# JJanai/slowflow

Measured on AMD Instinct MI355X. Metric: Mpix*solver-iters/s at 1024x436 (whole coarse-to-fine path), higher is better.
Workload: dtype f32

## Files before the change

### slowflow_amd/csrc/api.hip

```cpp
#include <algorithm>
#include <cmath>
#include <cstring>
#include <memory>
#include <mutex>

#include "sfa_internal.h"

#pragma clang fp contract(off)

namespace sfa {

thread_local std::string g_thread_err;

#ifndef SFA_RELEASE
Switches g_switches;
#endif
#ifndef SFA_RELEASE
static const char *const kSwitchNames[Switches::N] = {
    "SFA_SOR_CHAIN", "SFA_SOR_BAND", "SFA_SOR_F", "SFA_SOR_CH", "SFA_SOR_LEAD", "SFA_CHAIN_LDS", "SFA_RB_TILE", "SFA_WARP_ALLJ", "SFA_NO_WARP_SMOOTH",
    "SFA_ASSEMBLE_GENERIC", "SFA_EXACT_DIV", "SFA_ASM_XCD", "SFA_NO_DIRECT_OPERANDS", "SFA_NO_UV_ALIAS", "SFA_DEBUG_ACTIVE", "SFA_UNFUSED", "SFA_SHARE_SOR",
    "SFA_PYRAMID_UNFUSED", "SFA_CUT_DISCHARGE", "SFA_CUT_INNER", "SFA_CUT_SUPER", "SFA_CUT_TAIL_INNER", "SFA_CUT_PER", "SFA_CUT_TAIL_PER", "SFA_CUT_TAIL_SUPER",
    "SFA_CUT_DEBUG", "SFA_CUT_NO_TAIL", "SFA_CUT_TAIL", "SFA_NO_EXACT_BREAK"};
static int set_switch(const char *name, const char *value) {
    for (int i = 0; i < Switches::N; i++)
        if (!strcmp(name, kSwitchNames[i])) {
            g_switches.given[i] = value != nullptr;
            g_switches.value[i] = value ? atoi(value) : 0;
            return SFA_OK;
        }
    return SFA_ERR_ARG;
}
static void switches_from_environment() {
    static std::once_flag once;
    std::call_once(once, [] {
        const char *d = getenv("SFA_DEBUG");
        if (!d || atoi(d) == 0) return;
        for (int i = 0; i < Switches::N; i++)
            if (const char *e = getenv(kSwitchNames[i])) (void)set_switch(kSwitchNames[i], e);
    });
}
#else
static void switches_from_environment() {}
#endif

int set_error(sfa_ctx *ctx, int code, const char *fmt, ...) {
// ... 58 lines not shown
    float *warp(int s, int sp1) const { return base + off_warp + (long)(s + sp1) * 3 * pl; }
    float *frame(int f) const { return pbase + 2 * pl + (long)f * 3 * pl; }
    float *tmp() const { return base + off_tmp; }
    Geo geo() const { return Geo{w, h, pitch, pl, es, nb, WMask::first(nb), nullptr}; }
    Geo geo(const WMask &active) const { return Geo{w, h, pitch, pl, es, nb, active, nullptr}; }
    static long persistent_floats(int pitch, int h, int ref) { return (long)pitch * h * (2 + (2L * ref + 1) * 3); }
    static long transient_floats(int pitch, int h, int ref, bool fused) {
        return (long)pitch * h * ((P_COUNT - 2) + 2 * ref + (2L * ref + 1) * 3 + (fused ? 0 : 2L * ref * 2 * 24));
    }
    void layout(float *transient, float *persistent, int w_, int h_, int lstride_, int ref_, int nb_, long es_, bool fused_) {
        base = transient; pbase = persistent; w = w_; h = h_; pitch = dev_pitch(w_); lstride = lstride_; ref = ref_; F = 2 * ref_ + 1; nb = nb_; es = es_; fused = fused_;
        pl = (long)pitch * h;
        off_masks = (long)(P_COUNT - 2) * pl;
        off_warp = off_masks + 2L * ref * pl;
        off_stacks = off_warp + (2L * ref + 1) * 3 * pl;
        off_tmp = off_warp;
    }
};

struct ChannelWeights { const float *dev = nullptr; long pl = 0, es = 0; int pitch = 0, stride0 = 0; };

static const float *pair_image(const Level &L, int s, int sp1) { return (s + sp1 - L.ref == 0) ? L.frame(s + sp1) : L.warp(s, sp1); }

static bool get_derivatives(sfa_ctx *c, const Level &L, const sfa_params &p, const Geo &g, const bool need_toref[2 * SFA_MAX_REF], bool with_smoothness = false) {
    const int ref = L.ref;
    WarpJobs J;
    J.n = 0;
    for (int f = p.one_direction ? ref + 1 : 0; f <= 2 * ref; f++) {
        if (f == ref) continue;
        const int s = f < ref ? f : f - 1;
        J.job[J.n++] = WarpJob{L.frame(f) - L.base, L.warp(f < ref ? f : f - 1, f < ref ? 0 : 1) - L.base, L.mask(s) - L.base, f - ref};
    }
    const bool smoothed = with_smoothness && L.fused &&
                          launch_warp_smooth(c, g, J, L.base, L.plane(P_WX), L.plane(P_WY), p.smoothing, L.plane(P_SH), L.plane(P_SV), L.plane(P_DPSIS), p.alpha, pen(p.robust_reg));
    if (!smoothed) launch_warp_jobs(c, g, J, L.base, L.plane(P_WX), L.plane(P_WY));
    for (int s = p.one_direction ? ref : 0; s < 2 * ref; s++) {
        if (L.fused) continue;
        const float *w_s = pair_image(L, s, 0), *w_sp1 = pair_image(L, s, 1);
        launch_deriv_stack(c, g, L.stack(s, 0), w_s, w_sp1, L.es, L.es);
        if (need_toref[s]) {
            if (s < ref) launch_deriv_stack(c, g, L.stack(s, 1), w_s, L.frame(ref), L.es, L.es);
            else         launch_deriv_stack(c, g, L.stack(s, 1), L.frame(ref), w_sp1, L.es, L.es);
        }
    }
    return smoothed;
}

static int optimize_occlusions(sfa_ctx *c, const Level &L, const sfa_params &p, const Geo &g, DevMem &scratch) {
    const int ref = L.ref;
    const size_t n = (size_t)L.nb * L.pl;
    SFA_TRY(scratch.alloc(c, (2 + kCutWorkPlanes) * n * sizeof(float)));
    float *d0 = scratch.f(), *d1 = d0 + n, *work = d1 + n;
    OccArgs oa;
    memset(&oa, 0, sizeof oa);
// ... 43 lines not shown
    AssembleArgs aa;
    memset(&aa, 0, sizeof aa);
    bool need_toref[2 * SFA_MAX_REF] = {false};
    for (int s = 0; s < ref; s++) {
        if (!p.one_direction) {
            if (p.rho[ref - 1 - s] > 0)
                aa.t[aa.n++] = Term{L.off_stacks + ((long)s * 2 + 0) * 24 * L.pl, L.off_masks + (long)s * L.pl, p.rho[ref - 1 - s] * delta_over3,
                                    p.rho[ref - 1 - s] * gamma_over3, (float)(s - ref), 0};
            if (p.omega[ref - 1 - s] > 0) {
                aa.t[aa.n++] = Term{L.off_stacks + ((long)s * 2 + 1) * 24 * L.pl, L.off_masks + (long)s * L.pl, p.omega[ref - 1 - s] * delta_over3,
                                    p.omega[ref - 1 - s] * gamma_over3, (float)(s - ref), 1};
                need_toref[s] = true;
            }
        }
        if (p.rho[s] > 0)
            aa.t[aa.n++] = Term{L.off_stacks + ((long)(ref + s) * 2 + 0) * 24 * L.pl, L.off_masks + (long)(ref + s) * L.pl, p.rho[s] * delta_over3,
                                p.rho[s] * gamma_over3, (float)s, 0};
        if (p.omega[s] > 0) {
            aa.t[aa.n++] = Term{L.off_stacks + ((long)(ref + s) * 2 + 1) * 24 * L.pl, L.off_masks + (long)(ref + s) * L.pl, p.omega[s] * delta_over3,
                                p.omega[s] * gamma_over3, (float)(s + 1), 1};
            need_toref[ref + s] = true;
        }
    }
    for (int t = 0; t < aa.n; t++) {
        Term &T = aa.t[t];
        const int slot = (int)((T.mask_off - L.off_masks) / L.pl);
        const float *i1 = pair_image(L, slot, 0), *i2 = pair_image(L, slot, 1);
        if (T.is_ref) { if (slot < ref) i2 = L.frame(ref); else i1 = L.frame(ref); }
        T.i1_off = i1 - L.base; T.i2_off = i2 - L.base; T.backward = slot < ref;
    }
    aa.data_norm = data_norm; aa.one_direction = p.one_direction;
    for (int t = 0; t < aa.n; t++)
        if (aa.t[t].is_ref && aa.t[t].s == 0) return set_error(c, SFA_ERR_REF_FRAME, "Frame compared to reference frame is the reference frame itself!");
    aa.dt_norm = p.dataterm_norm;
    aa.color = pen(p.robust_color); aa.grad = pen(p.robust_grad);
    aa.chw = cw.dev; aa.chw_pl = cw.pl; aa.chw_es = cw.es; aa.chw_pitch = cw.pitch; aa.chw_stride0 = cw.stride0; aa.lstride = L.lstride;
    aa.accumulate = 0; aa.do_laplacian = 1;

    const bool use_thres_in = p.thres_inner > 0, use_thres_out = p.thres_outer > 0;
    double *red = c->d_red;
    const double npx = (double)L.h * L.w;
    constexpr int kLag = kMaskLag, kRing = kMaskRing;
    const bool dbg = sw_given(Switches::DEBUG_ACTIVE);
    g.amask = c->d_amask;
    float *const dfa = use_thres_out && !sw_given(Switches::NO_EXACT_BREAK) ? L.plane(P_A11) : nullptr, *const dfb = dfa ? L.plane(P_A12) : nullptr;
    float *const ifa = use_thres_in && !sw_given(Switches::NO_EXACT_BREAK) ? L.plane(P_A11) : nullptr, *const ifb = ifa ? L.plane(P_A12) : nullptr;
    SFA_HIP(c, hipMemsetAsync(c->d_last, 0, sizeof(LastBlock), c->stream));
    launch_set_mask(c, all);

    for (int alter = 0; alter < p.niter_alter; alter++) {
        active = all;
        g.active = active;
        if (use_thres_out && alter > 0) launch_set_mask(c, all);
        bool smoothed = get_derivatives(c, L, p, g, need_toref, uv_alias);
        if (alter > 0 && p.occlusion_reasoning && !p.one_direction) SFA_TRY(optimize_occlusions(c, L, p, g, cut_scratch));
        if (alter > 0 && p.occlusion_reasoning && occ_log)
            launch_copy_planes(c, g, occ_log + (long)alter * L.pl, L.plane(P_OCC), 1, (long)p.niter_alter * L.pl, L.es);
        for (int outer = 0; outer < p.niter_outer; outer++) {
            if (use_thres_out && outer >= kLag) {
                const int slot = (outer - kLag) % kRing;
                SFA_HIP(c, hipEventSynchronize(c->ev_mask[slot]));
                for (int i = 0; i < kMaskWords; i++) active.w[i] = *(volatile unsigned long long *)&c->h_amask[slot].w[i];
                if (!active.any()) break;
            }
            if (dbg) fprintf(stderr, "level %dx%d alter %d outer %d known active %d\n", L.w, L.h, alter, outer, active.count());
            g.active = active;
            if (outer > 0) smoothed = get_derivatives(c, L, p, g, need_toref, uv_alias);
            if (!L.fused) launch_mask_weight(c, g, L.mask(0), L.plane(P_OCC), data_norm, ref, p.one_direction);
            const bool red_black = p.sor_order == 1;
            const bool direct_outer = L.fused && !red_black && !sw_given(Switches::NO_DIRECT_OPERANDS);
            if (!direct_outer) launch_zero_planes(c, g, L.plane(P_DU), 2);
            WMask in_active = active, outer_done = WMask::none();
            for (int inner = 0; inner < p.niter_inner; inner++) {
                Geo gi = g;
                gi.active = in_active;
                const bool direct = direct_outer;
                const bool decide_in = use_thres_in && inner + 1 < p.niter_inner && ifa;
                const bool first_zero = direct && inner == 0;
                if (!first_zero) {
                    launch_copy_planes(c, gi, L.plane(P_ODU), L.plane(P_DU), 2, L.es, L.es);
                }
                if (!(smoothed && inner == 0))
                    launch_smoothness(c, gi, p.smoothing, L.plane(P_SH), L.plane(P_SV), UU, VV, L.plane(P_DPSIS), p.alpha,
                                      pen(p.robust_reg));
                aa.op = SorOperandOut();
                aa.zero_duv = first_zero ? 1 : 0;
                if (direct) SFA_TRY(sor_operand_target(c, sorws, gi, p.niter_solver, &aa.op));
                if (L.fused)
                    SFA_TRY(launch_assemble_images(c, gi, aa, L.base, L.plane(P_A11), L.plane(P_A12), L.plane(P_A22), L.plane(P_B1), L.plane(P_B2), L.plane(P_DU),
                                                   L.plane(P_DV), UU, VV, L.plane(P_SH), L.plane(P_SV), L.plane(P_OCC)));
// ... 1079 lines not shown
```

### slowflow_amd/csrc/kernels.hip

```cpp
#include "sfa_device.h"

#pragma clang fp contract(off)

namespace sfa {

__device__ __forceinline__ float psi_vec(const PenaltyDev &p, float xsq) {
    const float e2 = p.eps * p.eps;
    switch (p.id) {
    case 0: return 1.0f;
    case 2: return __fdiv_rn(1.0f, 2.0f * e2 + xsq);
    case 3: {
        float out = __fdiv_rn(1.0f, 2.0f * sqrt_rn(xsq + e2));
        if (sqrt_rn(xsq) > p.trunc) out = 0.0f;
        return out;
    }
    case 4: {
        float t = e2 + xsq;
        t = t * t;
        return __fdiv_rn(e2 + 2.0f * xsq, t);
    }
    default: return __fdiv_rn(1.0f, 2.0f * sqrt_rn(xsq + e2));
    }
}
__device__ __forceinline__ float psi_scalar(const PenaltyDev &p, float xsq) {
// ... 6 lines not shown
        if (sqrt_rn(xsq) > p.trunc) return 0.0f;
        return __fdiv_rn(1.0f, 2.0f * sqrt_rn(xsq + e2f));
    case 4: {
        float t = (float)(e2d + (double)xsq);
        t = t * t;
        return (float)((e2d + (double)(2.0f * xsq)) / (double)t);
    }
    default: return (float)(1.0 / (2.0 * __dsqrt_rn((double)xsq + e2d)));
    }
}

__global__ void k_warp(float *__restrict__ dst3, float *__restrict__ mask, const float *__restrict__ src3, const float *__restrict__ wx,
                       const float *__restrict__ wy, Geo g, int factor, long src_es) {
    const int b = blockIdx.z;
    if (!elem_active(g, b)) return;
    const int x = blockIdx.x * BX + threadIdx.x, y = blockIdx.y * BY + threadIdx.y;
    if (x >= g.w || y >= g.h) return;
    dst3 += b * g.es; wx += b * g.es; wy += b * g.es; src3 += b * src_es;
    const size_t o = (size_t)y * g.pitch + x;
    if (factor == 0) {
        for (int k = 0; k < 3; k++) dst3[k * g.pl + o] = src3[k * g.pl + o];
        return;
    }
    const float xx = x + factor * wx[o];
    const float yy = y + factor * wy[o];
    const int xi = floor_to_int_x86(xx), yi = floor_to_int_x86(yy);
    const float dx = xx - xi, dy = yy - yi;
    if (mask) mask[b * g.es + o] = (xx >= 0 && xx <= g.w - 1 && yy >= 0 && yy <= g.h - 1) ? 1.0f : 0.0f;
    const int x1 = clampi(xi, 0, g.w - 1), x2 = clampi(xi + 1, 0, g.w - 1);
    const int y1 = clampi(yi, 0, g.h - 1), y2 = clampi(yi + 1, 0, g.h - 1);
    const float ax = 1.0f - dx, ay = 1.0f - dy;
    for (int k = 0; k < 3; k++) {
        const float *s = src3 + k * g.pl;
        dst3[k * g.pl + o] = s[(size_t)y1 * g.pitch + x1] * ax * ay + s[(size_t)y1 * g.pitch + x2] * dx * ay
                           + s[(size_t)y2 * g.pitch + x1] * ax * dy + s[(size_t)y2 * g.pitch + x2] * dx * dy;
    }
}
template <bool ALLJ>
__global__ void k_warp_jobs(WarpJobs J, float *__restrict__ base, const float *__restrict__ wx, const float *__restrict__ wy, Geo g) {
    const int b = ALLJ ? blockIdx.z : blockIdx.z / J.n, j0 = ALLJ ? 0 : blockIdx.z % J.n;
    if (!elem_active(g, b)) return;
    const int x = blockIdx.x * BX + threadIdx.x, y = blockIdx.y * BY + threadIdx.y;
    if (x >= g.w || y >= g.h) return;
    const long eb = b * g.es;
    const size_t o = (size_t)y * g.pitch + x;
    const float fx0 = wx[eb + o], fy0 = wy[eb + o];
    for (int j = j0; j <= (ALLJ ? J.n - 1 : j0); j++) {
        const int factor = J.job[j].factor;
        const float *src3 = base + eb + J.job[j].src_off;
        float *dst3 = base + eb + J.job[j].dst_off;
        const float xx = x + factor * fx0;
        const float yy = y + factor * fy0;
        const int xi = floor_to_int_x86(xx), yi = floor_to_int_x86(yy);
        const float dx = xx - xi, dy = yy - yi;
        if (J.job[j].mask_off >= 0) base[eb + J.job[j].mask_off + o] = (xx >= 0 && xx <= g.w - 1 && yy >= 0 && yy <= g.h - 1) ? 1.0f : 0.0f;
        const int x1 = clampi(xi, 0, g.w - 1), x2 = clampi(xi + 1, 0, g.w - 1);
        const int y1 = clampi(yi, 0, g.h - 1), y2 = clampi(yi + 1, 0, g.h - 1);
        const float ax = 1.0f - dx, ay = 1.0f - dy;
        float out[3];
#pragma unroll
        for (int k = 0; k < 3; k++) {
            const float *s = src3 + k * g.pl;
            out[k] = s[(size_t)y1 * g.pitch + x1] * ax * ay + s[(size_t)y1 * g.pitch + x2] * dx * ay
                   + s[(size_t)y2 * g.pitch + x1] * ax * dy + s[(size_t)y2 * g.pitch + x2] * dx * dy;
        }
#pragma unroll
        for (int k = 0; k < 3; k++) dst3[k * g.pl + o] = out[k];
    }
}
void launch_warp_jobs(sfa_ctx *c, const Geo &g, const WarpJobs &J, float *base, const float *wx, const float *wy) {
    if (J.n <= 0) return;
    const bool allj = sw_int(Switches::WARP_ALLJ, 1) != 0;
    if (allj) hipLaunchKernelGGL(k_warp_jobs<true>, grid2d(g), block2d(), 0, c->stream, J, base, wx, wy, g);
    else hipLaunchKernelGGL(k_warp_jobs<false>, grid2d(g, J.n), block2d(), 0, c->stream, J, base, wx, wy, g);
}
void launch_warp(sfa_ctx *c, const Geo &g, float *dst3, float *mask, const float *src3, const float *wx, const float *wy, int factor, long src_es) {
    hipLaunchKernelGGL(k_warp, grid2d(g), block2d(), 0, c->stream, dst3, mask, src3, wx, wy, g, factor, src_es);
}
// ... 315 lines not shown
    const unsigned pitch4 = 4u * (unsigned)g.pitch;
    const float *pu = uu_ + eb, *pv = vv_ + eb, *pd = dps_ + eb;
    for (int i = tid; i < SM_R * SM_W; i += 64 * WS_ROWS) {
        const int gx = x0 + i % SM_W, gy = y0 + i / SM_W;
        if (gx >= 0 && gx < g.w && gy >= 0 && gy < g.h) {
            const unsigned o4 = (unsigned)gy * pitch4 + 4u * (unsigned)gx;
            tU[i] = ld(pu, o4); tV[i] = ld(pv, o4); tD[i] = ld(pd, o4);
        }
    }
    __syncthreads();
    const SmTile uu{tU, x0, y0}, vv{tV, x0, y0}, dps{tD, x0, y0};
    const int w = g.w, h = g.h;
    const int x = x0 + 1 + threadIdx.x;
    sh += eb; sv += eb;
    for (int k = 0; k < SM_Y / WS_ROWS; k++) {
        const int y = y0 + 1 + threadIdx.y + WS_ROWS * k;
        if (x >= g.pitch || y >= h) continue;
        const unsigned o4 = (unsigned)y * pitch4 + 4u * (unsigned)x;
        if (x >= w) { st(sh, o4, 0.0f); st(sv, o4, 0.0f); continue; }
        const float fx0 = uu(x, y), fy0 = vv(x, y);
        auto gather = [&](int j, float(&out)[3]) {
            const int factor = J.job[j].factor;
            const float *src3 = base + eb + J.job[j].src_off;
            const float xx = x + factor * fx0;
            const float yy = y + factor * fy0;
            const int xi = floor_to_int_x86(xx), yi = floor_to_int_x86(yy);
            const float dx = xx - xi, dy = yy - yi;
            if (J.job[j].mask_off >= 0) st(base + eb + J.job[j].mask_off, o4, (xx >= 0 && xx <= g.w - 1 && yy >= 0 && yy <= g.h - 1) ? 1.0f : 0.0f);
            const int x1 = clampi(xi, 0, g.w - 1), x2 = clampi(xi + 1, 0, g.w - 1);
            const int y1 = clampi(yi, 0, g.h - 1), y2 = clampi(yi + 1, 0, g.h - 1);
            const float ax = 1.0f - dx, ay = 1.0f - dy;
            const unsigned r1 = (unsigned)y1 * pitch4, r2 = (unsigned)y2 * pitch4, c1 = 4u * (unsigned)x1, c2 = 4u * (unsigned)x2;
            const unsigned o11 = (SFA_X_WS & 1) ? o4 : r1 + c1, o12 = (SFA_X_WS & 1) ? o4 : r1 + c2, o21 = (SFA_X_WS & 1) ? o4 : r2 + c1, o22 = (SFA_X_WS & 1) ? o4 : r2 + c2;
#pragma unroll
            for (int ch = 0; ch < 3; ch++) {
                const float *sp = src3 + ch * g.pl;
                if (SFA_X_WS & 8) { out[ch] = ax * ay + dx * dy; continue; }
#if defined(SFA_WS_LDNT) && SFA_WS_LDNT
                auto ldn = [](const float *ubase, unsigned boff) { return __builtin_nontemporal_load(reinterpret_cast<const float *>(reinterpret_cast<const char *>(ubase) + boff)); };
                out[ch] = ldn(sp, o11) * ax * ay + ldn(sp, o12) * dx * ay + ldn(sp, o21) * ax * dy + ldn(sp, o22) * dx * dy;
#else
                out[ch] = ld(sp, o11) * ax * ay + ld(sp, o12) * dx * ay + ld(sp, o21) * ax * dy + ld(sp, o22) * dx * dy;
#endif
            }
        };
        auto put = [&](int j, const float(&out)[3]) {
            float *dst3 = base + eb + J.job[j].dst_off;
#pragma unroll
            for (int ch = 0; ch < 3; ch++) {
                if (SFA_X_WS & 4) continue;
                if (SFA_WS_NT) __builtin_nontemporal_store(out[ch], reinterpret_cast<float *>(reinterpret_cast<char *>(dst3 + ch * g.pl) + o4));
// ... 640 lines not shown
    } else { bx_ = blockIdx.x; by_ = blockIdx.y; b_ = blockIdx.z; }
    const int bx = __builtin_amdgcn_readfirstlane(bx_), by = __builtin_amdgcn_readfirstlane(by_), b = __builtin_amdgcn_readfirstlane(b_);
    if (a.op.sa && bx == 0 && by == 0) {
        for (int i = threadIdx.x; i < a.op.ntasks; i += NT) a.op.flags[(size_t)b * a.op.ntasks + i] = 0;
        if (b == 0 && threadIdx.x == 0) a.op.flags[(size_t)a.op.nb * a.op.ntasks] = 0;
    }
    if (!elem_active(g, b)) return;
#if SFA_ASM_STAGGER
    if (XT && blockIdx.x < 8u * 32u * 3u) {
        const unsigned j = blockIdx.x >> 3;
        const unsigned slot = SFA_ASM_STAGGER_MODE ? j % 3u : (j >> 5) % 3u;
        for (unsigned s_ = 0; s_ < slot * SFA_ASM_STAGGER; s_++) __builtin_amdgcn_s_sleep(100);
    }
#endif
    const int x0 = bx * DT_X - DT_H, y0 = by * TY - DT_H;
    const bool tile_in = SFA_TILE_FAST && x0 >= 0 && x0 + DT_W <= g.w && y0 >= 0 && y0 + TR <= g.h;
    const long eb = b * g.es;
    const int tx = threadIdx.x & 63;
    const int ty = __builtin_amdgcn_readfirstlane(threadIdx.x >> 6);
    const int x = x0 + DT_H + tx;
    const int dt_norm = FAST ? 1 : a.dt_norm;
    PenaltyDev pcolor = a.color, pgrad = a.grad;
    if (FAST) { pcolor.id = FAST; pgrad.id = FAST; }
    Acc A[NP];
    float u[NP], v[NP], wk[NP][3], fwd[NP], bwd[NP], oc[NP];
    bool ok[NP];
#pragma unroll
    for (int k = 0; k < NP; k++) {
        const int y = y0 + DT_H + ty + NR * k;
        ok[k] = x < g.w && y < g.h;
        A[k].a11 = A[k].a12 = A[k].a22 = A[k].b1 = A[k].b2 = 0.0f;
        u[k] = v[k] = 0.0f; fwd[k] = bwd[k] = 0.0f; oc[k] = 0.0f;
        wk[k][0] = wk[k][1] = wk[k][2] = 1.0f;
        if (!ok[k]) continue;
        const size_t o = (size_t)y * g.pitch + x;
        if (!ZUV) { u[k] = du[eb + o]; v[k] = dv[eb + o]; }
        if (!FAST && a.chw) {
            const unsigned lin = (unsigned)y * (unsigned)a.lstride + (unsigned)x;
            const unsigned r0 = lin / (unsigned)a.chw_stride0, c0 = lin % (unsigned)a.chw_stride0;
            const float *cw = a.chw + b * a.chw_es + r0 * a.chw_pitch + c0;
            wk[k][0] = cw[0]; wk[k][1] = cw[a.chw_pl]; wk[k][2] = cw[2 * a.chw_pl];
        }
        if (!(SFA_X_AI & 128)) oc[k] = occ[eb + o];
    }
    constexpr int QM = DT_W / 4, Q1 = AW1 / 4;
    const bool need_g = a.do_laplacian || a.op.sa;
    auto stage_epilogue_operands = [&]() {
        if (!need_g) return;
        for (int i0 = 0; i0 < NGQ; i0 += NT) {
            const int item = i0 + (int)threadIdx.x;
            const int q = item % QM, row = (item / QM) % GR, pl = item / (QM * GR);
            const int gy = y0 + DT_H - 1 + row, gx = x0 + 4 * q;
            const float *src = pl == 0 ? uu : pl == 1 ? vv : pl == 2 ? sh : sv;
            if (!(SFA_X_AI & 32) && item < NGQ && gy >= 0 && gy < g.h && gx >= 0 && gx + 3 < g.pitch && (pl >= 2 || a.do_laplacian))
                dma16(src + eb + (size_t)gy * g.pitch + gx, lds_addr(lds + 4 * (i0 + 64 * ty)));
        }
    };
    AT_MARK(13);
    if (a.n == 0) stage_epilogue_operands();
    float mk2[2][NP];
    for (int t = 0; t < a.n; t++) {
        const Term &T = a.t[t];
        const int ub = kAsmPair ? t & 1 : 0;
        float(*sM)[NM] = sM2 + 3 * ub;
        float(*sZ)[NM] = sZ2 + 3 * ub;
        if (ub == 0) {
        AT_MARK(0);
        if (t > 0) __syncthreads();
        AT_MARK(1);
        SFA_PRIO(SFA_PRIO_STAGE);
        const int npair = kAsmPair && t + 1 < a.n ? 2 : 1;
        constexpr int NSQ = 3 * TR * QM, NSI = (NSQ + 63) / 64;
        const Term &T0 = a.t[t], &T1 = a.t[t + npair - 1];
        const int from_a = npair == 2 ? (T1.i1_off == T0.i1_off ? 0 : T1.i1_off == T0.i2_off ? 1 : 2) : 0;
        const int from_b = npair == 2 ? (T1.i2_off == T0.i1_off ? 0 : T1.i2_off == T0.i2_off ? 1 : 2) : 0;
        const long set_src[4] = {T0.i1_off, T0.i2_off, T1.i1_off, T1.i2_off};
        const int set_dst[4] = {0, ZOFF, 3 * NM, ZOFF + 3 * NM};
        const float *set_base[4];
#pragma unroll
        for (int set = 0; set < 4; set++) set_base[set] = base + eb + set_src[set];
        const bool own_a = npair == 2 && from_a == 2, own_b = npair == 2 && from_b == 2;
        for (int part = ty; part < NSI; part += NR) {
            const int k = part * 64 + tx;
            const int q = k % QM, ly = (k / QM) % TR, ch = k / (QM * TR);
            const int gy = y0 + ly, gx = x0 + 4 * q;
            if (!(SFA_X_AI & 1) && k < NSQ && gy >= 0 && gy < g.h && gx >= 0 && gx + 3 < g.w) {
                const unsigned po = 4u * ((unsigned)ch * (unsigned)g.pl + (unsigned)gy * (unsigned)g.pitch + (unsigned)gx);
                const unsigned ld = lds_addr(lds + 256 * part);
                dma16s(set_base[0], po, ld + 4u * set_dst[0]);
                dma16s(set_base[1], po, ld + 4u * set_dst[1]);
                if (own_a) dma16s(set_base[2], po, ld + 4u * set_dst[2]);
                if (own_b) dma16s(set_base[3], po, ld + 4u * set_dst[3]);
            }
        }
#pragma unroll
        for (int k = 0; k < NP; k++) {
            const size_t o = (size_t)(y0 + DT_H + ty + NR * k) * g.pitch + x;
            mk2[0][k] = ok[k] && !(SFA_X_AI & 128) ? base[eb + T0.mask_off + o] : 0.0f;
            mk2[1][k] = npair == 2 ? (ok[k] && !(SFA_X_AI & 128) ? base[eb + T1.mask_off + o] : 0.0f) : mk2[0][k];
        }
        AT_MARK(2);
        asm volatile("s_waitcnt vmcnt(0)" ::: "memory");
#pragma unroll
        for (int k = 0; k < NP; k++) {
            asm volatile("" : "+v"(mk2[0][k]), "+v"(mk2[1][k]), "+v"(oc[k]));
            if (!FAST) asm volatile("" : "+v"(wk[k][0]), "+v"(wk[k][1]), "+v"(wk[k][2]));
            if (!ZUV) asm volatile("" : "+v"(u[k]), "+v"(v[k]));
        }
        AT_MARK(3);
        if (SFA_ASM_DMA_BARRIER || kAsmPair) __syncthreads();
        AT_MARK(4);
        if (t == 0) {
#pragma unroll
            for (int k = 0; k < NP; k++) {
                float factor = (oc[k] == 0.0f) ? 1.0f : 0.0f;
                factor = (1 + factor) * a.data_norm;
                bwd[k] = __fdiv_rn((oc[k] >= 0.0f) ? 1.0f : 0.0f, factor);
                fwd[k] = __fdiv_rn((oc[k] <= 0.0f) ? 1.0f : 0.0f, factor);
            }
        }
        if (tile_in) {
            for (int item = threadIdx.x; item < ((SFA_X_AI & 2) ? 0 : NSQ); item += NT) {
                auto quad = [&](int lds_off) { return *reinterpret_cast<const float4 *>(lds + lds_off + 4 * item); };
                auto convert = [&](const float4 &va, const float4 &vb, int lds_off) {
                    *reinterpret_cast<float4 *>(lds + lds_off + 4 * item) =
                        make_float4(0.5f * (vb.x + va.x), 0.5f * (vb.y + va.y), 0.5f * (vb.z + va.z), 0.5f * (vb.w + va.w));
                    *reinterpret_cast<float4 *>(lds + ZOFF + lds_off + 4 * item) = make_float4(va.x - vb.x, va.y - vb.y, va.z - vb.z, va.w - vb.w);
                };
                const float4 a0 = quad(0), b0 = quad(ZOFF);
                if (npair == 2) {
                    const float4 a1 = from_a == 0 ? a0 : from_a == 1 ? b0 : quad(3 * NM);
                    const float4 b1 = from_b == 0 ? a0 : from_b == 1 ? b0 : quad(ZOFF + 3 * NM);
                    convert(a1, b1, 3 * NM);
                }
                convert(a0, b0, 0);
            }
        } else
        for (int item = threadIdx.x; item < ((SFA_X_AI & 2) ? 0 : NSQ); item += NT) {
            const int q = item % QM, ly = (item / QM) % TR, ch = item / (QM * TR);
            const int gy = y0 + ly, gx = x0 + 4 * q;
            if (gy < 0 || gy >= g.h) continue;
            const bool interior = gx >= 0 && gx + 3 < g.w;
// ... 126 lines not shown
                };
                read_taps(0); read_taps(1);
                __builtin_amdgcn_sched_barrier(0);
                filters(0);
                __builtin_amdgcn_sched_barrier(0);
                read_taps(2);
                __builtin_amdgcn_sched_barrier(0);
                filters(1); filters(2);
            } else {
                const int xl = x0 + DT_H + txl, xc_ = xl < g.w ? xl : g.w - 1;
#pragma unroll
                for (int ch = 0; ch < 3; ch++) {
                    const Tile1Acc X{sX[ch], x0, y0 + 2}, Y{sY[ch], x0, y0 + 2};
                    const TileAcc Z{sZ[ch], x0, y0};
                    p.ixy[ch] = d5y(X, xc_, y, g.h);
                    p.iyy[ch] = d5y(Y, xc_, y, g.h);
                    p.iyz[ch] = d5y(Z, xc_, y, g.h);
                    p.ix[ch] = sX[ch][c]; p.iy[ch] = sY[ch][c]; p.iz[ch] = sZ[ch][cz];
                    p.ixx[ch] = d5x_in<AW1>(sX[ch], c);
                    p.ixz[ch] = d5x_in<DT_W>(sZ[ch], cz);
                }
            }
            if (!ok[k]) continue;
            float m = mk2[ub][k];
            if (!a.one_direction || !T.backward) m = T.backward ? 1.0f * bwd[k] * m : 1.0f * fwd[k] * m;
            if (SFA_X_AI & 16) {
                for (int ch = 0; ch < 3; ch++) {
                    A[k].a11 += p.ix[ch] + p.ixx[ch] + m; A[k].a12 += p.iy[ch] + p.ixy[ch]; A[k].a22 += p.iz[ch] + p.iyy[ch]; A[k].b1 += p.ixz[ch]; A[k].b2 += p.iyz[ch];
                }
            } else if (T.is_ref) term_ref<ZUV, FAST != 0>(A[k], p, m, u[k], v[k], T.hd, T.hg, T.s, dt_norm, pcolor, pgrad, a.chain_ok != 0);
            else          term_succ<ZUV, FAST != 0>(A[k], p, m, u[k], v[k], T.hd, T.hg, T.s, dt_norm, pcolor, pgrad, a.chain_ok != 0);
        }
    }
    float4(*tA)[67] = reinterpret_cast<float4(*)[67]>(lds + NGF);
    float4(*tB)[67] = tA + TY;
    float2(*tX)[69] = reinterpret_cast<float2(*)[69]>(tB + TY);
    AT_MARK(0);
    if (need_g) {
        asm volatile("s_waitcnt vmcnt(0)" ::: "memory");
        __syncthreads();
    }
    AT_MARK(9);
    SFA_PRIO(SFA_PRIO_STAGE);
    const Tile1Acc U{lds, x0, y0 + DT_H - 1}, V{lds + GR * DT_W, x0, y0 + DT_H - 1}, Hh{lds + 2 * GR * DT_W, x0, y0 + DT_H - 1},
        Wv{lds + 3 * GR * DT_W, x0, y0 + DT_H - 1};
#pragma unroll
    for (int k = 0; k < NP; k++) {
        if (!ok[k]) continue;
// ... 35 lines not shown
        const size_t e = (size_t)b * a.op.ent + (size_t)(c + r + a.op.G) * a.op.RP + (r + a.op.G);
        if (SFA_X_AI & 64) continue;
        const float2 xv = tX[rl][cl];
        unsigned long long xu;
        __builtin_memcpy(&xu, &xv, 8);
#if defined(SFA_ASM_NT) && SFA_ASM_NT
        typedef float v4f_ __attribute__((ext_vector_type(4)));
        const float4 qa = tA[rl][cl], qb = tB[rl][cl];
        __builtin_nontemporal_store((v4f_){qa.x, qa.y, qa.z, qa.w}, reinterpret_cast<v4f_ *>(a.op.sa + e));
        __builtin_nontemporal_store((v4f_){qb.x, qb.y, qb.z, qb.w}, reinterpret_cast<v4f_ *>(a.op.sb + e));
        __builtin_nontemporal_store(xu, a.op.x + e);
#else
        a.op.sa[e] = tA[rl][cl];
        a.op.sb[e] = tB[rl][cl];
        a.op.x[e] = xu;
#endif
    }
#ifdef SFA_ASM_TIMING
    AT_MARK(12);
    if ((threadIdx.x & 63) == 0 && (bx + 3 * by + 7 * b) % 61 == 0)
        for (int i = 0; i < 14; i++) atomicAdd(&g_asm_timing[i], at_acc[i]);
#endif
}
int launch_assemble_images(sfa_ctx *c, const Geo &g, const AssembleArgs &a_in, const float *base, float *a11, float *a12, float *a22, float *b1, float *b2,
                           const float *du, const float *dv, const float *uu, const float *vv, const float *sh, const float *sv, const float *occ) {
    AssembleArgs a = a_in;
    if ((unsigned long long)g.pl * 12ull >= (1ull << 32)) return set_error(c, SFA_ERR_ARG, "k_assemble_images: plane of %ld entries is beyond the kernel's 32-bit offsets", g.pl);
    const bool prof = c->profile && c->ev2_used + 2 <= c->ev2.size();
    if (prof) (void)hipEventRecord(c->ev2[c->ev2_used], c->stream);
    auto is_modl1 = [](int id) { return id != 0 && id != 2 && id != 3 && id != 4; };
    const bool foldable = a.dt_norm == 1 && !a.chw && !sw_given(Switches::ASSEMBLE_GENERIC);
    const int fast = !foldable ? 0 : (is_modl1(a.color.id) && is_modl1(a.grad.id)) ? 1 : (a.color.id == 2 && a.grad.id == 2) ? 2 : 0;
    {
        auto in = [](float v, float lo, float hi) { return v >= lo && v <= hi; };
        const float elo = fast == 2 ? 1.0f / 1024 : 1.0f / 1048576, ehi = fast == 2 ? 1024.0f : 1048576.0f, hlo = fast == 2 ? 1.0f / 4096 : 1.0f / 65536;
        bool okp = fast != 0 && in(a.data_norm, 1.0f / 256, 256.0f) && in(a.color.eps, elo, ehi) && in(a.grad.eps, elo, ehi);
        for (int t = 0; t < a.n && okp; t++) okp = (a.t[t].hd == 0.0f || in(a.t[t].hd, hlo, 65536.0f)) && (a.t[t].hg == 0.0f || in(a.t[t].hg, hlo, 65536.0f));
        a.chain_ok = okp && !sw_given(Switches::EXACT_DIV) ? 1 : 0;
    }
    const dim3 grid_((g.w + DT_X - 1) / DT_X, (g.h + kAsmTY - 1) / kAsmTY, g.nb);
    const bool xcd_env = sw_int(Switches::ASM_XCD, 1) != 0;
    const long ntiles = (long)grid_.x * grid_.y * grid_.z;
    const bool xcd = xcd_env && ntiles >= 64 && ntiles < (1l << 30);
    const XcdTiles xt{(int)grid_.x, (int)grid_.y, (int)((ntiles + 7) / 8)};
    const dim3 grid1_(8u * (unsigned)xt.chunk, 1, 1);
#define SFA_LAUNCH_AI(ZUV_, FAST_)                                                                                                                      \
    do {                                                                                                                                                \
        if (xcd) hipLaunchKernelGGL((k_assemble_images<kAsmTY, kAsmNT, kAsmMinWaves, ZUV_, FAST_, true>), grid1_, dim3(kAsmNT), 0, c->stream, a, base, a11, a12, a22, b1, b2, du, dv, uu, vv, sh, sv, occ, g, xt); \
        else hipLaunchKernelGGL((k_assemble_images<kAsmTY, kAsmNT, kAsmMinWaves, ZUV_, FAST_, false>), grid_, dim3(kAsmNT), 0, c->stream, a, base, a11, a12, a22, b1, b2, du, dv, uu, vv, sh, sv, occ, g, xt); \
    } while (0)
    if (a.zero_duv) { if (fast == 1) SFA_LAUNCH_AI(true, 1); else if (fast == 2) SFA_LAUNCH_AI(true, 2); else SFA_LAUNCH_AI(true, 0); }
    else            { if (fast == 1) SFA_LAUNCH_AI(false, 1); else if (fast == 2) SFA_LAUNCH_AI(false, 2); else SFA_LAUNCH_AI(false, 0); }
#undef SFA_LAUNCH_AI
    if (prof) {
        (void)hipEventRecord(c->ev2[c->ev2_used + 1], c->stream);
        c->ev2_used += 2;
        c->asm_pixel_terms += (double)g.w * g.h * g.nb * a.n;
    }
    return SFA_OK;
}

// ... 725 lines not shown
```

### slowflow_amd/csrc/sfa_device.h

```cpp
#pragma once
#include "sfa_internal.h"

#pragma clang fp contract(off)

namespace sfa {

#define BX 64
#define BY 4

static inline dim3 grid2d(const Geo &g, int zmul = 1) { return dim3((g.w + BX - 1) / BX, (g.h + BY - 1) / BY, g.nb * zmul); }
static inline dim3 block2d() { return dim3(BX, BY, 1); }

__device__ __forceinline__ bool elem_active(const WMask &active, const unsigned long long *amask, int b) {
    const unsigned long long m = amask ? (active.w[b >> 6] & amask[b >> 6]) : active.w[b >> 6];
    return (m >> (b & 63)) & 1ull;
}
__device__ __forceinline__ bool elem_active(const Geo &g, int b) { return elem_active(g.active, g.amask, b); }
__device__ __forceinline__ int clampi(int a, int lo, int hi) { return a < lo ? lo : (a > hi ? hi : a); }
__device__ __forceinline__ int floor_to_int_x86(float v) {
    const float f = floorf(v);
    return (f >= -2147483648.0f && f < 2147483648.0f) ? (int)f : (-2147483647 - 1);
}

#define C5_0 (1.0f / 12.0f)
#define C5_1 (-8.0f / 12.0f)
#define C5_2 (-0.0f)
#define C5_3 (8.0f / 12.0f)
#define C5_4 (-(1.0f / 12.0f))
#define C3_0 (-0.5f)
#define C3_1 (-0.0f)
#define C3_2 (0.5f)

__device__ __forceinline__ float tap5(float m2, float m1, float c, float p1, float p2) {
#if defined(SFA_X_NO_CENTRE_TAP)
    return C5_0 * m2 + C5_1 * m1 + C5_3 * p1 + C5_4 * p2;
#else
    return C5_0 * m2 + C5_1 * m1 + C5_2 * c + C5_3 * p1 + C5_4 * p2;
#endif
}

template <class F>
__device__ __forceinline__ float d5x(F f, int x, int y, int w) {
    return tap5(f(clampi(x - 2, 0, w - 1), y), f(clampi(x - 1, 0, w - 1), y), f(x, y), f(clampi(x + 1, 0, w - 1), y), f(clampi(x + 2, 0, w - 1), y));
}
template <class F>
// ... 39 lines not shown
```

### slowflow_amd/csrc/sfa_internal.h

```cpp
#pragma once
#include <hip/hip_runtime.h>

#include <cstdarg>
#include <cstdio>
#include <string>
#include <vector>

#include "../../include/slowflow_amd.h"

#pragma clang fp contract(off)

namespace sfa {

constexpr int kMaskWords = 2;
constexpr int kMaxBatch = 64 * kMaskWords;
struct WMask {
    unsigned long long w[kMaskWords];
    __host__ __device__ bool test(int b) const { return (w[b >> 6] >> (b & 63)) & 1ull; }
    __host__ __device__ void clear(int b) { w[b >> 6] &= ~(1ull << (b & 63)); }
    __host__ __device__ void set(int b) { w[b >> 6] |= 1ull << (b & 63); }
    __host__ __device__ bool any() const { unsigned long long o = 0; for (int i = 0; i < kMaskWords; i++) o |= w[i]; return o != 0; }
    __host__ __device__ bool operator==(const WMask &o) const { bool e = true; for (int i = 0; i < kMaskWords; i++) e = e && w[i] == o.w[i]; return e; }
    __host__ __device__ bool operator!=(const WMask &o) const { return !(*this == o); }
    __host__ __device__ WMask operator&(const WMask &o) const { WMask r; for (int i = 0; i < kMaskWords; i++) r.w[i] = w[i] & o.w[i]; return r; }
// ... 43 lines not shown
    double sor_bytes = 0;
    std::vector<hipEvent_t> ev2;
    size_t ev2_used = 0;
    double asm_pixel_terms = 0;
    char sor_kernel[160] = {0};
    void *rb_tmp = nullptr;
    size_t rb_tmp_bytes = 0;
    hipEvent_t t0 = nullptr, t1 = nullptr;
    bool verbose_changes = false;
    int cu_count = 256;
};

namespace sfa {

constexpr int kRedDoubles = 1 << 20;

int set_error(sfa_ctx *ctx, int code, const char *fmt, ...);
extern thread_local std::string g_thread_err;

struct Switches {
    enum Id {
        SOR_CHAIN, SOR_BAND, SOR_F, SOR_CH, SOR_LEAD, CHAIN_LDS, RB_TILE, WARP_ALLJ, NO_WARP_SMOOTH, ASSEMBLE_GENERIC, EXACT_DIV, ASM_XCD, NO_DIRECT_OPERANDS,
        NO_UV_ALIAS, DEBUG_ACTIVE, UNFUSED, SHARE_SOR, PYRAMID_UNFUSED, CUT_DISCHARGE, CUT_INNER, CUT_SUPER, CUT_TAIL_INNER, CUT_PER, CUT_TAIL_PER, CUT_TAIL_SUPER,
        CUT_DEBUG, CUT_NO_TAIL, CUT_TAIL, NO_EXACT_BREAK, N
    };
    bool given[N] = {};
    int value[N] = {};
};
#ifdef SFA_RELEASE
#define SFA_FULL(...)
#else
#define SFA_FULL(...) __VA_ARGS__
#endif
#ifdef SFA_RELEASE
constexpr bool sw_given(Switches::Id) { return false; }
constexpr int sw_int(Switches::Id, int dflt) { return dflt; }
#else
extern Switches g_switches;
inline bool sw_given(Switches::Id i) { return g_switches.given[i]; }
inline int sw_int(Switches::Id i, int dflt) { return g_switches.given[i] ? g_switches.value[i] : dflt; }
#endif

#define SFA_HIP(ctx, call)                                                                         \
    do {                                                                                           \
        hipError_t _e = (call);                                                                    \
        if (_e != hipSuccess)                                                                      \
            return sfa::set_error((ctx), SFA_ERR_HIP, "%s failed: %s (%s:%d)", #call, hipGetErrorString(_e), __FILE__, __LINE__); \
// ... 39 lines not shown
void launch_warp(sfa_ctx *c, const Geo &g, float *dst3, float *mask, const float *src3, const float *wx, const float *wy, int factor,
                 long src_es );
void launch_deriv_stack(sfa_ctx *c, const Geo &g, float *out24, const float *I1, const float *I2, long es1, long es2);
void launch_convolve(sfa_ctx *c, const Geo &g, float *dst, const float *src, int order, int horiz, int nplanes);
void launch_dpsis(sfa_ctx *c, const Geo &g, float *dst, const float *im3, long im_es, float coef, const float avg[3], const float stdv[3], int hbit);
void launch_smoothness(sfa_ctx *c, const Geo &g, int method, float *sh, float *sv, const float *uu, const float *vv, const float *dpsis,
                       float alpha, PenaltyDev reg);
void launch_sub_laplacian(sfa_ctx *c, const Geo &g, float *dst, const float *src, const float *wh, const float *wv);
void launch_mask_weight(sfa_ctx *c, const Geo &g, float *masks, const float *occ, float data_norm, int ref, int one_direction);
void launch_fill(sfa_ctx *c, float *p, size_t n, float v);
void launch_division_chain(sfa_ctx *c, const float *a, const float *b, float *q_chain, float *q_exact, unsigned char *admitted, size_t n);
void launch_fill_planes(sfa_ctx *c, const Geo &g, float *p, int nplanes, float v);
void launch_zero_planes(sfa_ctx *c, const Geo &g, float *p, int nplanes);
void launch_outer_threshold(sfa_ctx *c, const Geo &g, const double *red, float thres, const float *dfa = nullptr, const float *dfb = nullptr);
void launch_set_mask(sfa_ctx *c, const WMask &v);

struct SorOperandOut {
    float4 *sa = nullptr, *sb = nullptr; unsigned long long *x = nullptr; unsigned *flags = nullptr;
    long ent = 0; int RP = 0, G = 0, ntasks = 0, nb = 0;
};
struct Term {
    long stack_off; long mask_off; float hd, hg, s; int is_ref;
    long i1_off, i2_off; int backward;
};
struct AssembleArgs {
    Term t[kMaxTerms];
    int n;
    int dt_norm;
    PenaltyDev color, grad;
    const float *chw; long chw_pl; long chw_es; int chw_pitch; int chw_stride0; int lstride;
    int accumulate;
    int do_laplacian;
    float data_norm; int one_direction;
    SorOperandOut op;
    int zero_duv;
    int chain_ok = 0;
};
void launch_assemble(sfa_ctx *c, const Geo &g, const AssembleArgs &a, const float *base , float *a11, float *a12,
                     float *a22, float *b1, float *b2, const float *du, const float *dv, const float *uu, const float *vv, const float *sh, const float *sv);

int launch_assemble_images(sfa_ctx *c, const Geo &g, const AssembleArgs &a, const float *base, float *a11, float *a12, float *a22, float *b1, float *b2,
                            const float *du, const float *dv, const float *uu, const float *vv, const float *sh, const float *sv, const float *occ);

void launch_smoothness_2f(sfa_ctx *c, const Geo &g, float *sh, float *sv, const float *uu, const float *vv, const float *dpsis, float half_alpha);
void launch_data_2f(sfa_ctx *c, const Geo &g, const float *D, const float *mask, const float *du, const float *dv, float *a11, float *a12, float *a22, float *b1,
                    float *b2, const float *wx, const float *wy, const float *sh, const float *sv, float hd, float hg);

struct OccSlot {
    long s1_off, s2_off;
    long r1_off, r2_off;
    long mask_off;
    float rho, omega;
    int label;
};
struct OccArgs { OccSlot slot[2 * SFA_MAX_REF]; int nslots; float hd, hg, penalty; PenaltyDev color, grad; };
void launch_occ_costs(sfa_ctx *c, const Geo &g, const OccArgs &a, const float *base, float *d0, float *d1, long d_es );
constexpr int kCutWorkPlanes = 13;
int run_grid_cut(sfa_ctx *c, const Geo &g, float *occ, long occ_es, const float *d0, const float *d1, float *work, float alpha);

void launch_update_inner(sfa_ctx *c, const Geo &g, float *uu, float *vv, const float *wx, const float *wy, const float *du, const float *dv,
// ... 44 lines not shown
```

Before: 260,700.

## Recompute warp validity masks from flow in assemble instead of storing them

```diff
diff --git a/slowflow_amd/csrc/api.hip b/slowflow_amd/csrc/api.hip
--- a/slowflow_amd/csrc/api.hip
+++ b/slowflow_amd/csrc/api.hip
@@ -20,7 +20,7 @@
     "SFA_SOR_CHAIN", "SFA_SOR_BAND", "SFA_SOR_F", "SFA_SOR_CH", "SFA_SOR_LEAD", "SFA_CHAIN_LDS", "SFA_RB_TILE", "SFA_WARP_ALLJ", "SFA_NO_WARP_SMOOTH",
     "SFA_ASSEMBLE_GENERIC", "SFA_EXACT_DIV", "SFA_ASM_XCD", "SFA_NO_DIRECT_OPERANDS", "SFA_NO_UV_ALIAS", "SFA_DEBUG_ACTIVE", "SFA_UNFUSED", "SFA_SHARE_SOR",
     "SFA_PYRAMID_UNFUSED", "SFA_CUT_DISCHARGE", "SFA_CUT_INNER", "SFA_CUT_SUPER", "SFA_CUT_TAIL_INNER", "SFA_CUT_PER", "SFA_CUT_TAIL_PER", "SFA_CUT_TAIL_SUPER",
-    "SFA_CUT_DEBUG", "SFA_CUT_NO_TAIL", "SFA_CUT_TAIL", "SFA_NO_EXACT_BREAK"};
+    "SFA_CUT_DEBUG", "SFA_CUT_NO_TAIL", "SFA_CUT_TAIL", "SFA_NO_EXACT_BREAK", "SFA_STORED_MASKS"};
 static int set_switch(const char *name, const char *value) {
     for (int i = 0; i < Switches::N; i++)
         if (!strcmp(name, kSwitchNames[i])) {
@@ -125,14 +125,15 @@
 
 static const float *pair_image(const Level &L, int s, int sp1) { return (s + sp1 - L.ref == 0) ? L.frame(s + sp1) : L.warp(s, sp1); }
 
-static bool get_derivatives(sfa_ctx *c, const Level &L, const sfa_params &p, const Geo &g, const bool need_toref[2 * SFA_MAX_REF], bool with_smoothness = false) {
+static bool get_derivatives(sfa_ctx *c, const Level &L, const sfa_params &p, const Geo &g, const bool need_toref[2 * SFA_MAX_REF], bool with_smoothness = false,
+                            bool store_masks = true) {
     const int ref = L.ref;
     WarpJobs J;
     J.n = 0;
     for (int f = p.one_direction ? ref + 1 : 0; f <= 2 * ref; f++) {
         if (f == ref) continue;
         const int s = f < ref ? f : f - 1;
-        J.job[J.n++] = WarpJob{L.frame(f) - L.base, L.warp(f < ref ? f : f - 1, f < ref ? 0 : 1) - L.base, L.mask(s) - L.base, f - ref};
+        J.job[J.n++] = WarpJob{L.frame(f) - L.base, L.warp(f < ref ? f : f - 1, f < ref ? 0 : 1) - L.base, store_masks ? L.mask(s) - L.base : -1L, f - ref};
     }
     const bool smoothed = with_smoothness && L.fused &&
                           launch_warp_smooth(c, g, J, L.base, L.plane(P_WX), L.plane(P_WY), p.smoothing, L.plane(P_SH), L.plane(P_SV), L.plane(P_DPSIS), p.alpha, pen(p.robust_reg));
@@ -222,13 +223,17 @@
             need_toref[ref + s] = true;
         }
     }
+    const bool flow_masks = L.fused && assemble_masks_from_flow();
     for (int t = 0; t < aa.n; t++) {
         Term &T = aa.t[t];
         const int slot = (int)((T.mask_off - L.off_masks) / L.pl);
         const float *i1 = pair_image(L, slot, 0), *i2 = pair_image(L, slot, 1);
         if (T.is_ref) { if (slot < ref) i2 = L.frame(ref); else i1 = L.frame(ref); }
         T.i1_off = i1 - L.base; T.i2_off = i2 - L.base; T.backward = slot < ref;
-    }
+        T.factor = (slot < ref ? slot : slot + 1) - ref;
+        T.mask_from_flow = flow_masks ? 1 : 0;
+    }
+    aa.wx = flow_masks ? L.plane(P_WX) : nullptr; aa.wy = flow_masks ? L.plane(P_WY) : nullptr;
     aa.data_norm = data_norm; aa.one_direction = p.one_direction;
     for (int t = 0; t < aa.n; t++)
         if (aa.t[t].is_ref && aa.t[t].s == 0) return set_error(c, SFA_ERR_REF_FRAME, "Frame compared to reference frame is the reference frame itself!");
@@ -252,8 +257,9 @@
         active = all;
         g.active = active;
         if (use_thres_out && alter > 0) launch_set_mask(c, all);
-        bool smoothed = get_derivatives(c, L, p, g, need_toref, uv_alias);
-        if (alter > 0 && p.occlusion_reasoning && !p.one_direction) SFA_TRY(optimize_occlusions(c, L, p, g, cut_scratch));
+        const bool occ_step = alter > 0 && p.occlusion_reasoning && !p.one_direction;
+        bool smoothed = get_derivatives(c, L, p, g, need_toref, uv_alias, !flow_masks || occ_step);
+        if (occ_step) SFA_TRY(optimize_occlusions(c, L, p, g, cut_scratch));
         if (alter > 0 && p.occlusion_reasoning && occ_log)
             launch_copy_planes(c, g, occ_log + (long)alter * L.pl, L.plane(P_OCC), 1, (long)p.niter_alter * L.pl, L.es);
         for (int outer = 0; outer < p.niter_outer; outer++) {
@@ -265,7 +271,7 @@
             }
             if (dbg) fprintf(stderr, "level %dx%d alter %d outer %d known active %d\n", L.w, L.h, alter, outer, active.count());
             g.active = active;
-            if (outer > 0) smoothed = get_derivatives(c, L, p, g, need_toref, uv_alias);
+            if (outer > 0) smoothed = get_derivatives(c, L, p, g, need_toref, uv_alias, !flow_masks);
             if (!L.fused) launch_mask_weight(c, g, L.mask(0), L.plane(P_OCC), data_norm, ref, p.one_direction);
             const bool red_black = p.sor_order == 1;
             const bool direct_outer = L.fused && !red_black && !sw_given(Switches::NO_DIRECT_OPERANDS);
diff --git a/slowflow_amd/csrc/kernels.hip b/slowflow_amd/csrc/kernels.hip
--- a/slowflow_amd/csrc/kernels.hip
+++ b/slowflow_amd/csrc/kernels.hip
@@ -52,11 +52,11 @@
         for (int k = 0; k < 3; k++) dst3[k * g.pl + o] = src3[k * g.pl + o];
         return;
     }
-    const float xx = x + factor * wx[o];
-    const float yy = y + factor * wy[o];
+    const float xx = warp_coord(x, factor, wx[o]);
+    const float yy = warp_coord(y, factor, wy[o]);
     const int xi = floor_to_int_x86(xx), yi = floor_to_int_x86(yy);
     const float dx = xx - xi, dy = yy - yi;
-    if (mask) mask[b * g.es + o] = (xx >= 0 && xx <= g.w - 1 && yy >= 0 && yy <= g.h - 1) ? 1.0f : 0.0f;
+    if (mask) mask[b * g.es + o] = warp_inside(xx, yy, g.w, g.h) ? 1.0f : 0.0f;
     const int x1 = clampi(xi, 0, g.w - 1), x2 = clampi(xi + 1, 0, g.w - 1);
     const int y1 = clampi(yi, 0, g.h - 1), y2 = clampi(yi + 1, 0, g.h - 1);
     const float ax = 1.0f - dx, ay = 1.0f - dy;
@@ -79,11 +79,11 @@
         const int factor = J.job[j].factor;
         const float *src3 = base + eb + J.job[j].src_off;
         float *dst3 = base + eb + J.job[j].dst_off;
-        const float xx = x + factor * fx0;
-        const float yy = y + factor * fy0;
+        const float xx = warp_coord(x, factor, fx0);
+        const float yy = warp_coord(y, factor, fy0);
         const int xi = floor_to_int_x86(xx), yi = floor_to_int_x86(yy);
         const float dx = xx - xi, dy = yy - yi;
-        if (J.job[j].mask_off >= 0) base[eb + J.job[j].mask_off + o] = (xx >= 0 && xx <= g.w - 1 && yy >= 0 && yy <= g.h - 1) ? 1.0f : 0.0f;
+        if (J.job[j].mask_off >= 0) base[eb + J.job[j].mask_off + o] = warp_inside(xx, yy, g.w, g.h) ? 1.0f : 0.0f;
         const int x1 = clampi(xi, 0, g.w - 1), x2 = clampi(xi + 1, 0, g.w - 1);
         const int y1 = clampi(yi, 0, g.h - 1), y2 = clampi(yi + 1, 0, g.h - 1);
         const float ax = 1.0f - dx, ay = 1.0f - dy;
@@ -445,11 +445,11 @@
         auto gather = [&](int j, float(&out)[3]) {
             const int factor = J.job[j].factor;
             const float *src3 = base + eb + J.job[j].src_off;
-            const float xx = x + factor * fx0;
-            const float yy = y + factor * fy0;
+            const float xx = warp_coord(x, factor, fx0);
+            const float yy = warp_coord(y, factor, fy0);
             const int xi = floor_to_int_x86(xx), yi = floor_to_int_x86(yy);
             const float dx = xx - xi, dy = yy - yi;
-            if (J.job[j].mask_off >= 0) st(base + eb + J.job[j].mask_off, o4, (xx >= 0 && xx <= g.w - 1 && yy >= 0 && yy <= g.h - 1) ? 1.0f : 0.0f);
+            if (J.job[j].mask_off >= 0 && !(SFA_X_WS & 64)) st(base + eb + J.job[j].mask_off, o4, warp_inside(xx, yy, g.w, g.h) ? 1.0f : 0.0f);
             const int x1 = clampi(xi, 0, g.w - 1), x2 = clampi(xi + 1, 0, g.w - 1);
             const int y1 = clampi(yi, 0, g.h - 1), y2 = clampi(yi + 1, 0, g.h - 1);
             const float ax = 1.0f - dx, ay = 1.0f - dy;
@@ -1136,15 +1136,23 @@
     const int dt_norm = FAST ? 1 : a.dt_norm;
     PenaltyDev pcolor = a.color, pgrad = a.grad;
     if (FAST) { pcolor.id = FAST; pgrad.id = FAST; }
+    const bool mflow = !kAsmPair && a.wx != nullptr;
     Acc A[NP];
-    float u[NP], v[NP], wk[NP][3], fwd[NP], bwd[NP], oc[NP];
+    float u[NP], v[NP], wk[NP][3], oc[NP];
     bool ok[NP];
+    auto mask_weight = [&](int backward, float ocv) -> float {
+        const bool on = backward ? ocv >= 0.0f : ocv <= 0.0f;
+        if (a.norm_ok) return on ? ((ocv == 0.0f) ? a.inv_2norm : a.inv_norm) : 0.0f;
+        float factor = (ocv == 0.0f) ? 1.0f : 0.0f;
+        factor = (1 + factor) * a.data_norm;
+        return __fdiv_rn(on ? 1.0f : 0.0f, factor);
+    };
 #pragma unroll
     for (int k = 0; k < NP; k++) {
         const int y = y0 + DT_H + ty + NR * k;
         ok[k] = x < g.w && y < g.h;
         A[k].a11 = A[k].a12 = A[k].a22 = A[k].b1 = A[k].b2 = 0.0f;
-        u[k] = v[k] = 0.0f; fwd[k] = bwd[k] = 0.0f; oc[k] = 0.0f;
+        u[k] = v[k] = 0.0f; oc[k] = 0.0f;
         wk[k][0] = wk[k][1] = wk[k][2] = 1.0f;
         if (!ok[k]) continue;
         const size_t o = (size_t)y * g.pitch + x;
@@ -1156,6 +1164,7 @@
             wk[k][0] = cw[0]; wk[k][1] = cw[a.chw_pl]; wk[k][2] = cw[2 * a.chw_pl];
         }
         if (!(SFA_X_AI & 128)) oc[k] = occ[eb + o];
+        if (mflow && !(SFA_X_AI & 128)) { A[k].b1 = a.wx[eb + o]; A[k].b2 = a.wy[eb + o]; }
     }
     constexpr int QM = DT_W / 4, Q1 = AW1 / 4;
     const bool need_g = a.do_laplacian || a.op.sa;
@@ -1173,6 +1182,10 @@
     AT_MARK(13);
     if (a.n == 0) stage_epilogue_operands();
     float mk2[2][NP];
+    unsigned mbits[NP];
+    static_assert(kMaxTerms <= 32, "one mask bit per term");
+#pragma unroll
+    for (int k = 0; k < NP; k++) mbits[k] = 0u;
     for (int t = 0; t < a.n; t++) {
         const Term &T = a.t[t];
         const int ub = kAsmPair ? t & 1 : 0;
@@ -1210,8 +1223,9 @@
 #pragma unroll
         for (int k = 0; k < NP; k++) {
             const size_t o = (size_t)(y0 + DT_H + ty + NR * k) * g.pitch + x;
-            mk2[0][k] = ok[k] && !(SFA_X_AI & 128) ? base[eb + T0.mask_off + o] : 0.0f;
-            mk2[1][k] = npair == 2 ? (ok[k] && !(SFA_X_AI & 128) ? base[eb + T1.mask_off + o] : 0.0f) : mk2[0][k];
+            const bool rd = ok[k] && !mflow && !(SFA_X_AI & 128);
+            mk2[0][k] = rd ? base[eb + T0.mask_off + o] : 0.0f;
+            mk2[1][k] = npair == 2 ? (rd ? base[eb + T1.mask_off + o] : 0.0f) : mk2[0][k];
         }
         AT_MARK(2);
         asm volatile("s_waitcnt vmcnt(0)" ::: "memory");
@@ -1227,11 +1241,24 @@
         if (t == 0) {
 #pragma unroll
             for (int k = 0; k < NP; k++) {
-                float factor = (oc[k] == 0.0f) ? 1.0f : 0.0f;
-                factor = (1 + factor) * a.data_norm;
-                bwd[k] = __fdiv_rn((oc[k] >= 0.0f) ? 1.0f : 0.0f, factor);
-                fwd[k] = __fdiv_rn((oc[k] <= 0.0f) ? 1.0f : 0.0f, factor);
-            }
+                if (mflow) {
+                    asm volatile("" : "+v"(A[k].b1), "+v"(A[k].b2));
+                    int xm = x, ym = y0 + DT_H + ty + NR * k, wm = g.w, hm = g.h;
+                    asm volatile("" : "+v"(xm), "+s"(ym), "+s"(wm), "+s"(hm));
+                    unsigned mb = 0u;
+#pragma unroll 1
+                    for (int tt = 0; tt < a.n; tt++) {
+                        const int wf = a.t[tt].factor;
+                        mb |= warp_inside(warp_coord(xm, wf, A[k].b1), warp_coord(ym, wf, A[k].b2), wm, hm) ? 1u << tt : 0u;
+                    }
+                    mbits[k] = mb;
+                    A[k].b1 = A[k].b2 = 0.0f;
+                }
+            }
+        }
+        if (!kAsmPair && !mflow) {
+#pragma unroll
+            for (int k = 0; k < NP; k++) mbits[k] = (mbits[k] & ~(1u << t)) | (mk2[0][k] != 0.0f ? 1u << t : 0u);
         }
         if (tile_in) {
             for (int item = threadIdx.x; item < ((SFA_X_AI & 2) ? 0 : NSQ); item += NT) {
@@ -1404,8 +1431,8 @@
                 }
             }
             if (!ok[k]) continue;
-            float m = mk2[ub][k];
-            if (!a.one_direction || !T.backward) m = T.backward ? 1.0f * bwd[k] * m : 1.0f * fwd[k] * m;
+            float m = kAsmPair ? mk2[ub][k] : ((mbits[k] >> t) & 1u) ? 1.0f : 0.0f;
+            if (!a.one_direction || !T.backward) m = 1.0f * mask_weight(T.backward, oc[k]) * m;
             if (SFA_X_AI & 16) {
                 for (int ch = 0; ch < 3; ch++) {
                     A[k].a11 += p.ix[ch] + p.ixx[ch] + m; A[k].a12 += p.iy[ch] + p.ixy[ch]; A[k].a22 += p.iz[ch] + p.iyy[ch]; A[k].b1 += p.ixz[ch]; A[k].b2 += p.iyz[ch];
@@ -1487,6 +1514,7 @@
         for (int i = 0; i < 14; i++) atomicAdd(&g_asm_timing[i], at_acc[i]);
 #endif
 }
+bool assemble_masks_from_flow() { return !kAsmPair && !sw_given(Switches::STORED_MASKS); }
 int launch_assemble_images(sfa_ctx *c, const Geo &g, const AssembleArgs &a_in, const float *base, float *a11, float *a12, float *a22, float *b1, float *b2,
                            const float *du, const float *dv, const float *uu, const float *vv, const float *sh, const float *sv, const float *occ) {
     AssembleArgs a = a_in;
@@ -1502,6 +1530,16 @@
         bool okp = fast != 0 && in(a.data_norm, 1.0f / 256, 256.0f) && in(a.color.eps, elo, ehi) && in(a.grad.eps, elo, ehi);
         for (int t = 0; t < a.n && okp; t++) okp = (a.t[t].hd == 0.0f || in(a.t[t].hd, hlo, 65536.0f)) && (a.t[t].hg == 0.0f || in(a.t[t].hg, hlo, 65536.0f));
         a.chain_ok = okp && !sw_given(Switches::EXACT_DIV) ? 1 : 0;
+        a.norm_ok = in(a.data_norm, 1.0f / 256, 256.0f) && !sw_given(Switches::EXACT_DIV) ? 1 : 0;
+        a.inv_norm = a.norm_ok ? 1.0f / a.data_norm : 0.0f;
+        a.inv_2norm = a.norm_ok ? 1.0f / ((1 + 1.0f) * a.data_norm) : 0.0f;
+    }
+    {
+        bool any = false, all = a.n > 0;
+        for (int t = 0; t < a.n; t++) { any = any || a.t[t].mask_from_flow; all = all && a.t[t].mask_from_flow; }
+        const bool flow = all && a.wx && a.wy && assemble_masks_from_flow();
+        if (any && !flow) return set_error(c, SFA_ERR_ARG, "k_assemble_images: masks from the flow need every term marked, wx / wy, and a build that forms them");
+        if (!flow) a.wx = a.wy = nullptr;
     }
     const dim3 grid_((g.w + DT_X - 1) / DT_X, (g.h + kAsmTY - 1) / kAsmTY, g.nb);
     const bool xcd_env = sw_int(Switches::ASM_XCD, 1) != 0;
diff --git a/slowflow_amd/csrc/sfa_device.h b/slowflow_amd/csrc/sfa_device.h
--- a/slowflow_amd/csrc/sfa_device.h
+++ b/slowflow_amd/csrc/sfa_device.h
@@ -21,6 +21,9 @@
     const float f = floorf(v);
     return (f >= -2147483648.0f && f < 2147483648.0f) ? (int)f : (-2147483647 - 1);
 }
+
+__device__ __forceinline__ float warp_coord(int x, int factor, float flow) { return x + factor * flow; }
+__device__ __forceinline__ bool warp_inside(float xx, float yy, int w, int h) { return xx >= 0 && xx <= w - 1 && yy >= 0 && yy <= h - 1; }
 
 #define C5_0 (1.0f / 12.0f)
 #define C5_1 (-8.0f / 12.0f)
diff --git a/slowflow_amd/csrc/sfa_internal.h b/slowflow_amd/csrc/sfa_internal.h
--- a/slowflow_amd/csrc/sfa_internal.h
+++ b/slowflow_amd/csrc/sfa_internal.h
@@ -89,7 +89,7 @@
     enum Id {
         SOR_CHAIN, SOR_BAND, SOR_F, SOR_CH, SOR_LEAD, CHAIN_LDS, RB_TILE, WARP_ALLJ, NO_WARP_SMOOTH, ASSEMBLE_GENERIC, EXACT_DIV, ASM_XCD, NO_DIRECT_OPERANDS,
         NO_UV_ALIAS, DEBUG_ACTIVE, UNFUSED, SHARE_SOR, PYRAMID_UNFUSED, CUT_DISCHARGE, CUT_INNER, CUT_SUPER, CUT_TAIL_INNER, CUT_PER, CUT_TAIL_PER, CUT_TAIL_SUPER,
-        CUT_DEBUG, CUT_NO_TAIL, CUT_TAIL, NO_EXACT_BREAK, N
+        CUT_DEBUG, CUT_NO_TAIL, CUT_TAIL, NO_EXACT_BREAK, STORED_MASKS, N
     };
     bool given[N] = {};
     int value[N] = {};
@@ -175,6 +175,7 @@
 struct Term {
     long stack_off; long mask_off; float hd, hg, s; int is_ref;
     long i1_off, i2_off; int backward;
+    int factor, mask_from_flow;
 };
 struct AssembleArgs {
     Term t[kMaxTerms];
@@ -188,7 +189,10 @@
     SorOperandOut op;
     int zero_duv;
     int chain_ok = 0;
-};
+    const float *wx = nullptr, *wy = nullptr;
+    float inv_norm = 0, inv_2norm = 0; int norm_ok = 0;
+};
+bool assemble_masks_from_flow();
 void launch_assemble(sfa_ctx *c, const Geo &g, const AssembleArgs &a, const float *base , float *a11, float *a12,
                      float *a22, float *b1, float *b2, const float *du, const float *dv, const float *uu, const float *vv, const float *sh, const float *sv);
 
```

After: 260,200 (median of 2 runs). No clear change (-0.2%).
